# Harrypotterrrr/DVD-GAN

Hardware: AMD Instinct MI355X
Metric: clips/sec per G+Ds+Dt step, 48x64x64 UCF-101 synth (higher is better)
Workload: dtype bf16; 1 GPU; UCF-101-shaped 101-class 48x64x64 clips, G+Ds+Dt hinge step, ch=32, k_sample=8, batch 64/GPU (BASELINE configs[1]); global_batch=64, parallelism=dp1

## Files before the change

### dvd_gan_amd/csrc/conv_common.h

```cpp
#pragma once
#include "common.h"

namespace dvdk {

constexpr int BM = 128, BN = 128, NT = 256;
constexpr int TILEB = BM * 80;
constexpr int WG_LD = 132;

__device__ __forceinline__ u32x4 relu16_f32(u32x4 v) {
    v.x = (int32_t)v.x < 0 ? 0u : v.x; v.y = (int32_t)v.y < 0 ? 0u : v.y;
    v.z = (int32_t)v.z < 0 ? 0u : v.z; v.w = (int32_t)v.w < 0 ? 0u : v.w;
    return v;
}
__device__ __forceinline__ uint32_t relu2_bf16(uint32_t v) {
    uint32_t m = ((v >> 15) & 0x00010001u) * 0xffffu;
    return v & ~m;
}
__device__ __forceinline__ u32x4 relu16_bf16(u32x4 v) {
    v.x = relu2_bf16(v.x); v.y = relu2_bf16(v.y); v.z = relu2_bf16(v.z); v.w = relu2_bf16(v.w);
    return v;
}
template <typename T> __device__ __forceinline__ u32x4 relu16(u32x4 v);
template <> __device__ __forceinline__ u32x4 relu16<float>(u32x4 v) { return relu16_f32(v); }
template <> __device__ __forceinline__ u32x4 relu16<bf16_t>(u32x4 v) { return relu16_bf16(v); }

__device__ __forceinline__ void grid_pos(int m, int H, int W, int logH, int logW, int& f, int& y, int& x) {
    if (logW >= 0) { x = m & (W - 1); y = (m >> logW) & (H - 1); f = m >> (logW + logH); }
    else { f = m / (H * W); const int r = m - f * (H * W); y = r / W; x = r - y * W; }
}

struct ConvK {
    const char* in; const char* w; const float* bias; const char* res; const char* mask;
    const char* wq;
    char* out; float* ws;
    int M, C, ldi, Cout, ldo, ldres, ldmask, res_up2;
    int T, H, W, logH, logW, Hin, Win;
    int kt, kh, kw, kchunks, nk, nsplit, tilesN;
    int up2, relu_in, act, out_f32;
    int nb32;
// ... 47 lines not shown
    a.x = pack2_bf16(v[0], v[1]); a.y = pack2_bf16(v[2], v[3]); a.z = pack2_bf16(v[4], v[5]); a.w = pack2_bf16(v[6], v[7]);
    __builtin_amdgcn_raw_buffer_store_b128(a, r, off, 0, 0);
}
template <> __device__ __forceinline__ void bst8<float>(__amdgpu_buffer_rsrc_t r, unsigned off, const float (&v)[8]) {
    u32x4 a = {__float_as_uint(v[0]), __float_as_uint(v[1]), __float_as_uint(v[2]), __float_as_uint(v[3])};
    u32x4 b = {__float_as_uint(v[4]), __float_as_uint(v[5]), __float_as_uint(v[6]), __float_as_uint(v[7])};
    __builtin_amdgcn_raw_buffer_store_b128(a, r, off, 0, 0);
    __builtin_amdgcn_raw_buffer_store_b128(b, r, off + 16, 0, 0);
}

template <int R, int D, class Stage, class Load, class Compute>
__device__ __forceinline__ void epi_run(Stage stage, Load load, Compute compute) {
#pragma unroll
    for (int i = 0; i < D && i < R; ++i) load(i);
#pragma unroll
    for (int i = 0; i < R; ++i) {
        if ((i & 3) == 0) stage(i >> 2);
        if (i + D < R) load(i + D);
        compute(i);
        if ((i & 3) == 3) __builtin_amdgcn_wave_barrier();
    }
}

template <int TM>
__device__ __forceinline__ bool splitk_combine(const ConvK& p, f32x16 (&acc)[TM][2], float* lds0, int lane, int z, int ltile) {
    constexpr unsigned kWaveBytes = TM * 2 * 4 * 1024;
    constexpr int kSc1 = 16;
    const int ns = p.nsplit;
    const int wave = threadIdx.x >> 6;
    const unsigned tileBytes = (blockDim.x >> 6) * kWaveBytes;
    const size_t tile = (size_t)ltile;
    const __amdgpu_buffer_rsrc_t rs = __builtin_amdgcn_make_buffer_rsrc(
        (void*)((char*)p.g.slabs + tile * ns * (size_t)tileBytes), 0, (unsigned)ns * tileBytes, 0x00020000);
    const unsigned lo = wave * kWaveBytes + lane * 16;
#pragma unroll
    for (int tm = 0; tm < TM; ++tm)
#pragma unroll
        for (int tn = 0; tn < 2; ++tn)
#pragma unroll
            for (int q = 0; q < 4; ++q) {
                const u32x4 v = {__float_as_uint(acc[tm][tn][4 * q]), __float_as_uint(acc[tm][tn][4 * q + 1]),
                                 __float_as_uint(acc[tm][tn][4 * q + 2]), __float_as_uint(acc[tm][tn][4 * q + 3])};
                __builtin_amdgcn_raw_buffer_store_b128(v, rs, z * tileBytes + lo + ((tm * 2 + tn) * 4 + q) * 1024, 0, kSc1);
            }
    asm volatile("s_waitcnt vmcnt(0)" ::: "memory");
    __syncthreads();
    if (threadIdx.x == 0)
        *reinterpret_cast<volatile unsigned*>(lds0) =
            __hip_atomic_fetch_add(p.g.tickets + tile, 1u, __ATOMIC_RELAXED, __HIP_MEMORY_SCOPE_AGENT);
    __syncthreads();
    const unsigned ticket = *reinterpret_cast<volatile unsigned*>(lds0);
    if (ticket != (unsigned)(ns - 1)) return false;
    __syncthreads();
    if (threadIdx.x == 0) __hip_atomic_store(p.g.tickets + tile, 0u, __ATOMIC_RELAXED, __HIP_MEMORY_SCOPE_AGENT);
    int s_begin = 0, s_end = ns;
    if (ns == 2) { s_begin = z ^ 1; s_end = s_begin + 1; }
    else {
        const f32x16 zacc = {0.f, 0.f, 0.f, 0.f, 0.f, 0.f, 0.f, 0.f, 0.f, 0.f, 0.f, 0.f, 0.f, 0.f, 0.f, 0.f};
#pragma unroll
        for (int tm = 0; tm < TM; ++tm)
#pragma unroll
            for (int tn = 0; tn < 2; ++tn) acc[tm][tn] = zacc;
    }
    u32x4 buf[2][4];
    auto issue = [&](int s, int g, u32x4 (&b)[4]) __attribute__((always_inline)) {
        const unsigned so = s < s_end ? (unsigned)s * tileBytes : kOOB;
#pragma unroll
        for (int i = 0; i < 4; ++i) b[i] = __builtin_amdgcn_raw_buffer_load_b128(rs, so + lo + (g * 4 + i) * 1024, 0, kSc1);
    };
    issue(s_begin, 0, buf[0]);
    for (int s = s_begin; s < s_end; ++s) {
#pragma unroll
        for (int g = 0; g < 2 * TM; ++g) {
            if (g + 1 < 2 * TM) issue(s, g + 1, buf[(g + 1) & 1]);
            else issue(s + 1, 0, buf[(g + 1) & 1]);
            __builtin_amdgcn_sched_barrier(0);
#pragma unroll
            for (int i = 0; i < 4; ++i) {
                const u32x4 v = buf[g & 1][i];
                f32x16& a = acc[g >> 1][g & 1];
                a[4 * i] += __uint_as_float(v.x); a[4 * i + 1] += __uint_as_float(v.y);
                a[4 * i + 2] += __uint_as_float(v.z); a[4 * i + 3] += __uint_as_float(v.w);
            }
            __builtin_amdgcn_sched_barrier(0);
        }
    }
    return true;
}

template <typename T, int TM, int DEEP = 0, bool COMBINE = true, class RelRow>
__device__ __forceinline__ void conv_epilogue(const ConvK& p, f32x16 (&acc)[TM][2], float* ep, int lane, int col, int z, int ltile,
                                              long long row0, RelRow relrow) {
    constexpr unsigned esz = sizeof(T);
    constexpr int R = 4 * TM;
    constexpr bool kB = sizeof(T) == 2;
    const int erow = lane >> 3, ecol = (lane & 7) * 8;
    const bool colv = col < p.Cout;
    const long long rows = (long long)p.M - row0;
    auto stage = [&](int tm) __attribute__((always_inline)) {
#pragma unroll
        for (int tn = 0; tn < 2; ++tn)
#pragma unroll
            for (int r = 0; r < 16; ++r)
                ep[((r & 3) + 8 * (r >> 2) + 4 * (lane >> 5)) * 64 + tn * 32 + (lane & 31)] = acc[tm][tn][r];
        __builtin_amdgcn_s_waitcnt(0xc07f);
        __builtin_amdgcn_wave_barrier();
    };
    auto staged = [&](int i, float (&v)[8]) __attribute__((always_inline)) {
        const f32x4 a = *reinterpret_cast<const f32x4*>(ep + ((i & 3) * 8 + erow) * 64 + ecol);
        const f32x4 b = *reinterpret_cast<const f32x4*>(ep + ((i & 3) * 8 + erow) * 64 + ecol + 4);
        v[0] = a[0]; v[1] = a[1]; v[2] = a[2]; v[3] = a[3]; v[4] = b[0]; v[5] = b[1]; v[6] = b[2]; v[7] = b[3];
    };
    auto rrow = [&](int i) __attribute__((always_inline)) -> int { return relrow(i >> 2, i & 3); };
    auto offs = [&](int rr, unsigned ld, unsigned eb, int c, bool ok) __attribute__((always_inline)) -> unsigned {
        return (rr >= 0 && ok) ? (unsigned)rr * (ld * eb) + (unsigned)c * eb : kOOB;
    };
    const int mode = p.g.mode;
#ifdef DVD_EXP_NOEPI
    return;
#endif
    if constexpr (COMBINE)
        if (mode != 0 && p.nsplit > 1 && !splitk_combine<TM>(p, acc, ep - (threadIdx.x >> 6) * (32 * 64), lane, z, ltile)) return;
    if (mode == 1) {
        constexpr int D = kB ? 3 : 1;
        const int h = p.g.h;
        const bool isr = col >= h;
        const int c2 = isr ? col - h : col;
// ... 286 lines not shown
```

### dvd_gan_amd/csrc/conv_gb.hip

```cpp
#include "conv_common.h"

namespace {

#ifndef DVD_GB_EPI_DEEP
#define DVD_GB_EPI_DEEP 0
#endif

constexpr unsigned kRowOOB = 0x80000000u, kStepOOB = 0x40000000u, kRangeCap = 0x3fffffffu;

template <int TM, int WN, int WMV, bool UP2> struct HaloGbCfg {
    static constexpr int PITCH = HaloGeo<UP2>::PITCH;
    static constexpr int NWAVE = WMV * WN;
    static constexpr int PH = WMV * TM * 2;
    static constexpr int HG = UP2 ? ((PH / 2 + 3) * PITCH + 15) / 16 : ((PH + 4) * PITCH + 15) / 16;
    static constexpr int HBYTES = HG * 1024;
    static constexpr int EPI = NWAVE * 32 * 64 * 4;
    static constexpr int LDSB = 2 * HBYTES + 1024 > EPI ? 2 * HBYTES + 1024 : EPI;
};

template <int TM, bool RELU, class LdA, class Next>
__device__ __forceinline__ void gb_step(f32x16 (&acc)[TM][2], const bf16x8 (&b)[2][2], LdA ldA, Next next) {
    constexpr int NU = 2 * TM;
#ifndef DVD_GB_ADEPTH
#define DVD_GB_ADEPTH 2
#endif
    constexpr int AD = DVD_GB_ADEPTH;
    bf16x8 a[NU];
#pragma unroll
    for (int u = 0; u < AD && u < NU; ++u) a[u] = ldA(u);
    __builtin_amdgcn_sched_barrier(0);
#pragma unroll
    for (int u = 0; u < NU; ++u) {
        if (u + AD < NU) a[u + AD] = ldA(u + AD);
        const int kk = u / TM, tm = u % TM;
        if constexpr (RELU) a[u] = __builtin_bit_cast(bf16x8, relu16_bf16(__builtin_bit_cast(u32x4, a[u])));
#pragma unroll
        for (int tn = 0; tn < 2; ++tn)
            acc[tm][tn] = __builtin_amdgcn_mfma_f32_32x32x16_bf16(a[u], b[kk][tn], acc[tm][tn], 0, 0, 0);
        __builtin_amdgcn_sched_barrier(0);
        if (u == 0) {
#ifndef DVD_EXP_NODMA
            next();
#endif
            __builtin_amdgcn_sched_barrier(0);
        }
    }
}

template <int TM, int WN, int WMV, bool RELU, bool UP2, int KS>
__device__ __forceinline__ void conv_halo_gb_tile(const ConvK& p, char* const smem, const int mt, const int nt, const int z, const int ltile) {
    using T = bf16_t;
    using G = HaloGeo<UP2>;
    using Cfg = HaloGbCfg<TM, WN, WMV, UP2>;
    constexpr int NWAVE = Cfg::NWAVE;
    constexpr int PITCH = G::PITCH;
    constexpr int BNt = WN * 64;
    constexpr int PH = Cfg::PH, HG = Cfg::HG, HBYTES = Cfg::HBYTES;
    constexpr int NH = (HG + NWAVE - 1) / NWAVE;
    constexpr int ntap2 = KS * KS;
    constexpr int pad = KS >> 1, cpad = (pad + 1) >> 1;
    constexpr int HWa = UP2 ? ((15 + pad) >> 1) + cpad + 1 : 16 + 2 * pad;
    constexpr int HHa = UP2 ? ((PH - 1 + pad) >> 1) + cpad + 1 : PH + 2 * pad;
    char* const hbuf0 = &smem[0];
    char* const dump = &smem[2 * HBYTES];
    const int tid = threadIdx.x, lane = tid & 63, wave = tid >> 6;
    const int wm = wave / WN, wn = wave % WN;
    const int n0 = nt * BNt;
    const int pw = p.W >> 4, ppf = pw * (p.H / PH);
    const int ft = mt / ppf, pidx = mt - ft * ppf;
    const int y0 = (pidx / pw) * PH, x0 = (pidx % pw) * 16;
    const int nouter = p.kchunks * p.kt;
    const int per = (nouter + p.nsplit - 1) / p.nsplit;
    const int oc_begin = z * per, oc_end = min(nouter, oc_begin + per);
    constexpr unsigned esz = 2;
    const int iy_lo = UP2 ? (y0 >> 1) - cpad : y0 - pad, ix_lo = UP2 ? (x0 >> 1) - cpad : x0 - pad;

    const int wu = __builtin_amdgcn_readfirstlane(wave);
    const int lrow = lane >> 2;
    const unsigned ldb = (unsigned)p.ldi * esz;
    const int tt = p.kt > 1 ? ft % p.T : 0;
    const int base_frame = max(0, ft - (p.kt >> 1));
    const size_t fbytes = (size_t)p.Hin * p.Win * ldb;
    const size_t base_b = (size_t)base_frame * fbytes;
    const size_t left_b = p.in_bytes - base_b;
    const __amdgpu_buffer_rsrc_t rin = __builtin_amdgcn_make_buffer_rsrc(
        (void*)(p.in + base_b), 0, left_b > kRangeCap ? kRangeCap : (unsigned)left_b, 0x00020000);
    const int nb32 = p.nb32;
    const __amdgpu_buffer_rsrc_t rwq = __builtin_amdgcn_make_buffer_rsrc(
        (void*)p.wq, 0, (unsigned)((size_t)p.kt * ntap2 * p.kchunks * nb32 * 2048), 0x00020000);
    auto hrow = [&](int i, int& hy, int& hx) __attribute__((always_inline)) {
        const int h = (i * NWAVE + wu) * 16 + lrow;
        hy = h / PITCH; hx = h - hy * PITCH;
    };
    unsigned hoff[NH];
#pragma unroll
    for (int i = 0; i < NH; ++i) {
        const int g = i * NWAVE + wu;
        int hy, hx;
        hrow(i, hy, hx);
        const int yin = iy_lo + hy, xin = ix_lo + hx;
        const int hq = (lane & 3) ^ G::sw(hy, hx);
        const bool ok = g < HG && hy < HHa && hx < HWa && (unsigned)yin < (unsigned)p.Hin && (unsigned)xin < (unsigned)p.Win;
        hoff[i] = ok ? (unsigned)(yin * p.Win + xin) * ldb + hq * 16 : kRowOOB;
    }
    const bool ragged = (p.C & 31) != 0;
    auto dmaH = [&](int hb, int cc_, int it_) __attribute__((always_inline)) {
        const int dt_ = it_ - (p.kt >> 1);
        const bool ok_ = (unsigned)(tt + dt_) < (unsigned)p.T || p.kt == 1;
        const unsigned ud_ = ok_ ? (unsigned)(ft + dt_ - base_frame) * (unsigned)fbytes + cc_ * 64 : kStepOOB;
        const bool part_ = ragged && cc_ == p.kchunks - 1;
#pragma unroll
        for (int i = 0; i < NH; ++i) {
            const int g = i * NWAVE + wu;
            char* dst_ = g < HG ? hbuf0 + hb * HBYTES + g * 1024 : dump;
            unsigned off_ = hoff[i] + ud_;
            if (part_) {
                int hy, hx;
                hrow(i, hy, hx);
                const int hq = (lane & 3) ^ G::sw(hy, hx);
                off_ = cc_ * 32 + hq * 8 < p.C ? off_ : kRowOOB;
            }
            dma16(rin, dst_, off_);
        }
    };
    const unsigned bvoff = (unsigned)(wn * 2 * 2048 + lane * 16);
    const unsigned bnt = (unsigned)(nt * (BNt / 32)) * 2048u;
    const unsigned brec = (unsigned)nb32 * 2048u;
    const unsigned tapstep = (unsigned)p.kchunks * brec;
    auto ldBq = [&](bf16x8 (&b)[2][2], unsigned rec) __attribute__((always_inline)) {
#pragma unroll
        for (int kk = 0; kk < 2; ++kk)
#pragma unroll
            for (int tn = 0; tn < 2; ++tn)
                b[kk][tn] = __builtin_bit_cast(bf16x8, __builtin_amdgcn_raw_buffer_load_b128(rwq, bvoff, rec + (unsigned)(tn * 2048 + kk * 1024), 0));
    };
    auto rec0 = [&](int cc_, int it_) __attribute__((always_inline)) -> unsigned {
        return ((unsigned)(it_ * ntap2) * p.kchunks + cc_) * brec + bnt;
    };

    f32x16 acc[TM][2];
    {
        const f32x16 zacc = {0.f, 0.f, 0.f, 0.f, 0.f, 0.f, 0.f, 0.f, 0.f, 0.f, 0.f, 0.f, 0.f, 0.f, 0.f, 0.f};
#pragma unroll
        for (int a = 0; a < TM; ++a)
#pragma unroll
            for (int b = 0; b < 2; ++b) acc[a][b] = zacc;
    }
    const int l31 = lane & 31, kh2 = lane >> 5;
    const int px = l31 & 15, py0 = wm * (TM * 2) + (l31 >> 4);
    constexpr int TMSTRIDE = (UP2 ? 1 : 2) * PITCH * 64;
#ifdef DVD_EXP_NOMAIN
    const int nouter_z = 0;
#else
    const int nouter_z = oc_end - oc_begin;
#endif
    if (nouter_z > 0) {
        int m_cc = oc_begin / p.kt, m_it = oc_begin - m_cc * p.kt;
        int h_cc = m_cc, h_it = m_it;
        bf16x8 bq0[2][2], bq1[2][2];
        unsigned rec = rec0(m_cc, m_it);
        dmaH(0, h_cc, h_it);
        if (++h_it == p.kt) { h_it = 0; ++h_cc; }
        ldBq(bq0, rec);
        __builtin_amdgcn_s_waitcnt(0x0070 | (0xf << 8));
        __builtin_amdgcn_s_barrier();
        int hb = 0, iy = 0, left = nouter_z;
        auto row = [&](bf16x8 (&b0)[2][2], bf16x8 (&b1)[2][2]) __attribute__((always_inline)) {
            const bool first = iy == 0, last = iy == KS - 1, more = left > 1;
            const int hy = UP2 ? ((py0 + iy - pad) >> 1) + cpad : py0 + iy;
            const char* const Arow = hbuf0 + hb * HBYTES + hy * (PITCH * 64);
#pragma unroll
            for (int ix = 0; ix < KS; ++ix) {
                const int hx = UP2 ? ((px + ix - pad) >> 1) + cpad : px + ix;
                const int swz = G::sw(hy, hx);
                const char* const Ah = Arow + hx * 64;
                auto ldA = [&](int u) __attribute__((always_inline)) -> bf16x8 {
                    const int kk = u / TM, tm = u % TM, slot = kk * 2 + kh2;
                    const int sl = (UP2 && (tm & 1)) ? (slot ^ 2) : slot;
                    return *reinterpret_cast<const bf16x8*>(Ah + tm * TMSTRIDE + ((sl ^ swz) << 4));
                };
                unsigned nrec = rec + tapstep;
                if (ix == KS - 1 && last) {
                    int n_cc = m_cc, n_it = m_it + 1;
                    if (n_it == p.kt) { n_it = 0; ++n_cc; }
                    nrec = more ? rec0(n_cc, n_it) : rec;
                    m_cc = n_cc; m_it = n_it;
                }
                auto next = [&]() __attribute__((always_inline)) {
                    ldBq((ix & 1) ? b0 : b1, nrec);
                    if (ix == 0 && first && more) { dmaH(hb ^ 1, h_cc, h_it); if (++h_it == p.kt) { h_it = 0; ++h_cc; } }
                };
                gb_step<TM, RELU>(acc, (ix & 1) ? b1 : b0, ldA, next);
                rec = nrec;
            }
            ++iy;
            if (last) {
                iy = 0; hb ^= 1; --left;
                if (more) {
#ifndef DVD_EXP_NOWAIT
                    __builtin_amdgcn_s_waitcnt(0xc07f);
#endif
#ifndef DVD_EXP_NOBAR
                    __builtin_amdgcn_s_barrier();
#endif
                }
            }
        };
        const int nrows = nouter_z * KS;
        int r = 0;
#pragma unroll 1
        for (; r + 1 < nrows; r += 2) { row(bq0, bq1); row(bq1, bq0); }
        if (r < nrows) row(bq0, bq1);
    }
    __syncthreads();

    float* ep = reinterpret_cast<float*>(&smem[0]) + wave * (32 * 64);
    const int ecol = (lane & 7) * 8, erow = lane >> 3;
    const long long frame_row0 = (long long)ft * (p.H * p.W);
    conv_epilogue<T, TM, DVD_GB_EPI_DEEP>(p, acc, ep, lane, n0 + wn * 64 + ecol, z, ltile, frame_row0, [&](int tm, int j) __attribute__((always_inline)) {
        const int pi = wm * (TM * 32) + tm * 32 + j * 8 + erow;
        return (y0 + (pi >> 4)) * p.W + x0 + (pi & 15);
    });
}

__device__ __forceinline__ int xcd_order(int bid, int nwg) {
    const int xcd = bid & 7, qd = nwg >> 3, rr = nwg & 7;
    return (xcd < rr ? xcd * (qd + 1) : rr * (qd + 1) + (xcd - rr) * qd) + (bid >> 3);
}
struct TileMN { int mt, nt; };
__device__ __forceinline__ TileMN tile_of(int nmajor, int tilesN, int t, int ntiles) {
    const int d = nmajor ? ntiles / tilesN : tilesN;
    const int q = t / d, r = t - q * d;
    TileMN o;
    o.mt = nmajor ? r : q; o.nt = nmajor ? q : r;
    return o;
}

template <int TM, int WN, int WMV, bool RELU, bool UP2, int KS>
__global__ __launch_bounds__(256, 2) void conv_halo_gb_kernel(ConvK p) {
    __shared__ __attribute__((aligned(16))) char smem[HaloGbCfg<TM, WN, WMV, UP2>::LDSB];
    const int bid = xcd_order(blockIdx.x, gridDim.x);
    const TileMN t = tile_of(p.nmajor, p.tilesN, bid, gridDim.x);
    conv_halo_gb_tile<TM, WN, WMV, RELU, UP2, KS>(p, smem, t.mt, t.nt, blockIdx.z, (int)blockIdx.x);
}

template <int TM, int S> struct HaloGbsCfg {
    static constexpr int PITCH = S + 4, FR = PITCH * PITCH;
    static constexpr int G = TM * 64 / (S * S);
    static constexpr int HG = (G * FR + 15) / 16;
    static constexpr int HBYTES = HG * 1024;
    static constexpr int EPI = 4 * 32 * 64 * 4;
    static constexpr int LDSB = 2 * HBYTES + 1024 > EPI ? 2 * HBYTES + 1024 : EPI;
};

template <int TM, int S, bool RELU, int KS>
__device__ __forceinline__ void conv_halo_gbs_tile(const ConvK& p, char* const smem, const int mt, const int nt, const int z, const int ltile) {
    using T = bf16_t;
    using Cfg = HaloGbsCfg<TM, S>;
    constexpr int WN = 2, NWAVE = 4, BNt = 128;
    constexpr int PITCH = Cfg::PITCH, FR = Cfg::FR, G = Cfg::G, HG = Cfg::HG, HBYTES = Cfg::HBYTES;
    constexpr int NH = (HG + NWAVE - 1) / NWAVE;
    constexpr int SS = S * S;
    constexpr int ntap2 = KS * KS, pad = KS >> 1, ext = S + 2 * pad;
    char* const hbuf0 = &smem[0];
    char* const dump = &smem[2 * HBYTES];
    const int tid = threadIdx.x, lane = tid & 63, wave = tid >> 6;
    const int wm = wave / WN, wn = wave % WN;
    const int n0 = nt * BNt;
    const int ft0 = mt * G, nframes = p.M / SS;
    const int per = (p.kchunks + p.nsplit - 1) / p.nsplit;
    const int cc_begin = z * per, cc_end = min(p.kchunks, cc_begin + per);
    constexpr unsigned esz = 2;

    const int wu = __builtin_amdgcn_readfirstlane(wave);
    const int lrow = lane >> 2;
    const unsigned ldb = (unsigned)p.ldi * esz;
    const size_t base_b = (size_t)ft0 * SS * ldb;
    const size_t left_b = p.in_bytes - base_b;
    const __amdgpu_buffer_rsrc_t rin = __builtin_amdgcn_make_buffer_rsrc(
        (void*)(p.in + base_b), 0, left_b > kRangeCap ? kRangeCap : (unsigned)left_b, 0x00020000);
    const int nb32 = p.nb32;
    const __amdgpu_buffer_rsrc_t rwq = __builtin_amdgcn_make_buffer_rsrc(
        (void*)p.wq, 0, (unsigned)((size_t)ntap2 * p.kchunks * nb32 * 2048), 0x00020000);
    auto hrow = [&](int i, int& fl, int& hy, int& hx) __attribute__((always_inline)) {
        const int h = (i * NWAVE + wu) * 16 + lrow;
        fl = h / FR;
        const int r = h - fl * FR;
        hy = r / PITCH; hx = r - hy * PITCH;
    };
    unsigned hoff[NH];
#pragma unroll
    for (int i = 0; i < NH; ++i) {
        const int g = i * NWAVE + wu;
        int fl, hy, hx;
        hrow(i, fl, hy, hx);
        const int yin = hy - pad, xin = hx - pad;
        const int hq = (lane & 3) ^ (hy & 3);
        const bool ok = g < HG && fl < G && ft0 + fl < nframes && hy < ext && hx < ext && (unsigned)yin < (unsigned)S && (unsigned)xin < (unsigned)S;
        hoff[i] = ok ? (unsigned)((fl * S + yin) * S + xin) * ldb + hq * 16 : kRowOOB;
    }
    const bool ragged = (p.C & 31) != 0;
    auto dmaH = [&](int hb, int cc_) __attribute__((always_inline)) {
        const bool part_ = ragged && cc_ == p.kchunks - 1;
#pragma unroll
        for (int i = 0; i < NH; ++i) {
            const int g = i * NWAVE + wu;
            char* dst_ = g < HG ? hbuf0 + hb * HBYTES + g * 1024 : dump;
            unsigned off_ = hoff[i] + cc_ * 64;
            if (part_) {
                int fl, hy, hx;
                hrow(i, fl, hy, hx);
                const int hq = (lane & 3) ^ (hy & 3);
                off_ = cc_ * 32 + hq * 8 < p.C ? off_ : kRowOOB;
            }
            dma16(rin, dst_, off_);
        }
    };
    const unsigned bvoff = (unsigned)(wn * 2 * 2048 + lane * 16);
    const unsigned bnt = (unsigned)(nt * (BNt / 32)) * 2048u;
    const unsigned brec = (unsigned)nb32 * 2048u;
    const unsigned tapstep = (unsigned)p.kchunks * brec;
    auto ldBq = [&](bf16x8 (&b)[2][2], unsigned rec) __attribute__((always_inline)) {
#pragma unroll
        for (int kk = 0; kk < 2; ++kk)
#pragma unroll
            for (int tn = 0; tn < 2; ++tn)
                b[kk][tn] = __builtin_bit_cast(bf16x8, __builtin_amdgcn_raw_buffer_load_b128(rwq, bvoff, rec + (unsigned)(tn * 2048 + kk * 1024), 0));
    };

    f32x16 acc[TM][2];
    {
        const f32x16 zacc = {0.f, 0.f, 0.f, 0.f, 0.f, 0.f, 0.f, 0.f, 0.f, 0.f, 0.f, 0.f, 0.f, 0.f, 0.f, 0.f};
#pragma unroll
        for (int a = 0; a < TM; ++a)
#pragma unroll
            for (int b = 0; b < 2; ++b) acc[a][b] = zacc;
    }
    const int l31 = lane & 31, kh2 = lane >> 5;
    const int pi0 = wm * (TM * 32) + l31;
    const int f0 = pi0 / SS, y0 = (pi0 % SS) / S, x0 = pi0 % S;
    const int arow0 = f0 * FR + y0 * PITCH + x0;
    auto tmoff = [](int tm) constexpr -> int { return S == 8 ? ((tm >> 1) * FR + (tm & 1) * 4 * PITCH) * 64 : tm * 2 * FR * 64; };
#ifdef DVD_EXP_NOMAIN
    const int nch = 0;
#else
    const int nch = cc_end - cc_begin;
#endif
    if (nch > 0) {
        unsigned rec = (unsigned)cc_begin * brec + bnt;
        bf16x8 bq0[2][2], bq1[2][2];
        dmaH(0, cc_begin);
        ldBq(bq0, rec);
        __builtin_amdgcn_s_waitcnt(0x0070 | (0xf << 8));
        __builtin_amdgcn_s_barrier();
        int hb = 0, iy = 0, cc = cc_begin;
        auto row = [&](bf16x8 (&b0)[2][2], bf16x8 (&b1)[2][2]) __attribute__((always_inline)) {
            const bool first = iy == 0, last = iy == KS - 1, more = cc + 1 < cc_end;
            const int swz = (y0 + iy) & 3;
            const char* const Arow = hbuf0 + hb * HBYTES + (arow0 + iy * PITCH) * 64;
#pragma unroll
            for (int ix = 0; ix < KS; ++ix) {
                const char* const Ah = Arow + ix * 64;
                auto ldA = [&](int u) __attribute__((always_inline)) -> bf16x8 {
                    const int kk = u / TM, tm = u % TM, slot = kk * 2 + kh2;
                    return *reinterpret_cast<const bf16x8*>(Ah + tmoff(tm) + ((slot ^ swz) << 4));
                };
                unsigned nrec = rec + tapstep;
                if (ix == KS - 1 && last) nrec = more ? (unsigned)(cc + 1) * brec + bnt : rec;
                auto next = [&]() __attribute__((always_inline)) {
                    ldBq((ix & 1) ? b0 : b1, nrec);
                    if (ix == 0 && first && more) dmaH(hb ^ 1, cc + 1);
                };
                gb_step<TM, RELU>(acc, (ix & 1) ? b1 : b0, ldA, next);
                rec = nrec;
            }
            ++iy;
            if (last) {
                iy = 0; hb ^= 1; ++cc;
                if (more) {
                    __builtin_amdgcn_s_waitcnt(0xc07f);
                    __builtin_amdgcn_s_barrier();
                }
            }
        };
        const int nrows = nch * KS;
        int r = 0;
#pragma unroll 1
        for (; r + 1 < nrows; r += 2) { row(bq0, bq1); row(bq1, bq0); }
        if (r < nrows) row(bq0, bq1);
    }
    __syncthreads();

    float* ep = reinterpret_cast<float*>(&smem[0]) + wave * (32 * 64);
    const int ecol = (lane & 7) * 8, erow = lane >> 3;
    const long long row0 = (long long)ft0 * SS;
    conv_epilogue<T, TM, DVD_GB_EPI_DEEP>(p, acc, ep, lane, n0 + wn * 64 + ecol, z, ltile, row0, [&](int tm, int j) __attribute__((always_inline)) {
        const int pi = wm * (TM * 32) + tm * 32 + j * 8 + erow;
        return row0 + pi < p.M ? pi : -1;
    });
}

template <int TM, int S, bool RELU, int KS>
__global__ __launch_bounds__(256, 2) void conv_halo_gbs_kernel(ConvK p) {
    __shared__ __attribute__((aligned(16))) char smem[HaloGbsCfg<TM, S>::LDSB];
    const int bid = xcd_order(blockIdx.x, gridDim.x);
    const TileMN t = tile_of(p.nmajor, p.tilesN, bid, gridDim.x);
    conv_halo_gbs_tile<TM, S, RELU, KS>(p, smem, t.mt, t.nt, blockIdx.z, (int)blockIdx.x);
}

template <class TileFn>
__device__ __forceinline__ void group_dispatch(const ConvGroup& grp, TileFn fn) {
    const int x = blockIdx.x & 7;
    int rem = blockIdx.x >> 3;
    auto share = [&](int m) __attribute__((always_inline)) -> int { const int w = grp.wgs[m]; return (w >> 3) + (x < (w & 7) ? 1 : 0); };
    const int m0 = grp.order[0], m1 = grp.n > 1 ? grp.order[1] : m0;
    const int s0 = share(m0), s1 = grp.n > 1 ? share(m1) : 0;
    const int h0 = min(grp.head, s0), h1 = min(grp.head, s1);
    int g = -1, off = 0;
    if (rem < h0) { g = m0; off = rem; }
    else if ((rem -= h0) < h1) { g = m1; off = rem; }
    else if ((rem -= h1) < s0 - h0) { g = m0; off = h0 + rem; }
    else if ((rem -= s0 - h0) < s1 - h1) { g = m1; off = h1 + rem; }
    else {
        rem -= s1 - h1;
        for (int k = 2; k < grp.n; ++k) {
            const int m = grp.order[k], s = share(m);
            if (rem < s) { g = m; off = rem; break; }
            rem -= s;
        }
    }
    if (g < 0) return;
    const int w = grp.wgs[g];
    const int local = x * (w >> 3) + min(x, w & 7) + off;
    const ConvK& p = grp.c[g];
    const int t = local / p.nsplit, z = local - t * p.nsplit;
    const TileMN mn = tile_of(p.nmajor, p.tilesN, t, w / p.nsplit);
    fn(p, mn.mt, mn.nt, z, t);
}

template <int TM, int WN, int WMV>
__global__ __launch_bounds__(256, 2) void conv_group_gb_kernel(ConvGroup grp) {
    __shared__ __attribute__((aligned(16))) char smem[HaloGbCfg<TM, WN, WMV, false>::LDSB];
    group_dispatch(grp, [&](const ConvK& p, int mt, int nt, int z, int t) __attribute__((always_inline)) {
        if (p.kh == 5) conv_halo_gb_tile<TM, WN, WMV, false, false, 5>(p, smem, mt, nt, z, t);
        else conv_halo_gb_tile<TM, WN, WMV, false, false, 3>(p, smem, mt, nt, z, t);
    });
}

template <int TM, int S>
__global__ __launch_bounds__(256, 2) void conv_group_gbs_kernel(ConvGroup grp) {
    __shared__ __attribute__((aligned(16))) char smem[HaloGbsCfg<TM, S>::LDSB];
    group_dispatch(grp, [&](const ConvK& p, int mt, int nt, int z, int t) __attribute__((always_inline)) {
        if (p.kh == 5) conv_halo_gbs_tile<TM, S, false, 5>(p, smem, mt, nt, z, t);
        else conv_halo_gbs_tile<TM, S, false, 3>(p, smem, mt, nt, z, t);
    });
}

}

namespace dvdk {
#define GB(R, C, KS, RL, UP) cv_key(CV_HALO_L2, 0, R, C, KS, RL, UP)
#define GBS(F, R, KS, RL) cv_key(F, 0, R, 128, KS, RL, 0)
static const ConvRow kGbRows[] = {
#ifdef DVD_GB_PROBE
    {GB(256, 128, 5, 0, 0), conv_halo_gb_kernel<4, 2, 2, false, false, 5>}, {GBS(CV_FRAME8, 128, 3, 0), conv_halo_gbs_kernel<2, 8, false, 3>},
#else
    {GB(256, 128, 3, 0, 0), conv_halo_gb_kernel<4, 2, 2, false, false, 3>}, {GB(256, 128, 3, 1, 0), conv_halo_gb_kernel<4, 2, 2, true, false, 3>},
    {GB(256, 128, 3, 0, 1), conv_halo_gb_kernel<4, 2, 2, false, true, 3>},  {GB(256, 128, 3, 1, 1), conv_halo_gb_kernel<4, 2, 2, true, true, 3>},
    {GB(256, 128, 5, 0, 0), conv_halo_gb_kernel<4, 2, 2, false, false, 5>}, {GB(256, 128, 5, 1, 0), conv_halo_gb_kernel<4, 2, 2, true, false, 5>},
    {GB(256, 128, 5, 0, 1), conv_halo_gb_kernel<4, 2, 2, false, true, 5>},  {GB(256, 128, 5, 1, 1), conv_halo_gb_kernel<4, 2, 2, true, true, 5>},
    {GB(128, 128, 3, 0, 0), conv_halo_gb_kernel<2, 2, 2, false, false, 3>}, {GB(128, 128, 3, 1, 0), conv_halo_gb_kernel<2, 2, 2, true, false, 3>},
    {GB(128, 128, 3, 0, 1), conv_halo_gb_kernel<2, 2, 2, false, true, 3>},  {GB(128, 128, 3, 1, 1), conv_halo_gb_kernel<2, 2, 2, true, true, 3>},
    {GB(128, 128, 5, 0, 0), conv_halo_gb_kernel<2, 2, 2, false, false, 5>}, {GB(128, 128, 5, 1, 0), conv_halo_gb_kernel<2, 2, 2, true, false, 5>},
// ... 27 lines not shown
```

Before: 146.4 clips/s.

## Switch halo conv kernels from 32x32x16 to 16x16x32 MFMA with remapped fragment rows

Replaces the 32x32x16 bf16 MFMA in the halo conv mainloops with 16x16x32 MFMA, using a compile-time row-permutation type that maps fragment rows to pixel positions. The A/B load addressing, accumulator layout, epilogue staging and split-k combine paths are made generic over the new accumulator type. It also raises launch-bounds occupancy to 3 blocks for small-TM variants, recomputes halo offsets on the fly for relu TM=4 to save registers, and uses packed i16 max for the bf16 relu. The goal is better MFMA throughput and occupancy, at the cost of more intricate layout logic and possible register pressure or LDS bank conflicts.

```diff
diff --git a/dvd_gan_amd/csrc/conv_common.h b/dvd_gan_amd/csrc/conv_common.h
--- a/dvd_gan_amd/csrc/conv_common.h
+++ b/dvd_gan_amd/csrc/conv_common.h
@@ -12,9 +12,9 @@
     v.z = (int32_t)v.z < 0 ? 0u : v.z; v.w = (int32_t)v.w < 0 ? 0u : v.w;
     return v;
 }
+typedef __attribute__((ext_vector_type(2))) short i16x2;
 __device__ __forceinline__ uint32_t relu2_bf16(uint32_t v) {
-    uint32_t m = ((v >> 15) & 0x00010001u) * 0xffffu;
-    return v & ~m;
+    return __builtin_bit_cast(uint32_t, __builtin_elementwise_max(__builtin_bit_cast(i16x2, v), i16x2{0, 0}));
 }
 __device__ __forceinline__ u32x4 relu16_bf16(u32x4 v) {
     v.x = relu2_bf16(v.x); v.y = relu2_bf16(v.y); v.z = relu2_bf16(v.z); v.w = relu2_bf16(v.w);
@@ -108,8 +108,68 @@
     }
 }
 
-template <int TM>
-__device__ __forceinline__ bool splitk_combine(const ConvK& p, f32x16 (&acc)[TM][2], float* lds0, int lane, int z, int ltile) {
+template <int B0, int B1, int B2, int B3, int B4> struct FragRows {
+    static constexpr int bit(int rid, int b) { return (rid >> b) & 1; }
+    static constexpr int pix(int h, int i) {
+        const int rid = h << 4 | i;
+        return bit(rid, B0) | bit(rid, B1) << 1 | bit(rid, B2) << 2 | bit(rid, B3) << 3 | bit(rid, B4) << 4;
+    }
+};
+using RowsHalo = FragRows<0, 1, 4, 2, 3>;
+using RowsUp2 = FragRows<0, 2, 3, 4, 1>;
+using RowsF8 = FragRows<0, 1, 2, 4, 3>;
+template <class Rows> struct Acc16 { f32x4 q[2][4]; };
+
+__device__ __forceinline__ void acc_zero(f32x16 (&t)[2]) {
+    const f32x16 z = {0.f, 0.f, 0.f, 0.f, 0.f, 0.f, 0.f, 0.f, 0.f, 0.f, 0.f, 0.f, 0.f, 0.f, 0.f, 0.f};
+    t[0] = z; t[1] = z;
+}
+template <class Rows> __device__ __forceinline__ void acc_zero(Acc16<Rows>& a) {
+    const f32x4 z = {0.f, 0.f, 0.f, 0.f};
+#pragma unroll
+    for (int g = 0; g < 8; ++g) a.q[g >> 2][g & 3] = z;
+}
+__device__ __forceinline__ u32x4 acc_quad(const f32x16 (&t)[2], int g) {
+    const f32x16& a = t[g >> 2];
+    const int q = g & 3;
+    return u32x4{__float_as_uint(a[4 * q]), __float_as_uint(a[4 * q + 1]), __float_as_uint(a[4 * q + 2]), __float_as_uint(a[4 * q + 3])};
+}
+template <class Rows> __device__ __forceinline__ u32x4 acc_quad(const Acc16<Rows>& a, int g) { return __builtin_bit_cast(u32x4, a.q[g >> 2][g & 3]); }
+__device__ __forceinline__ void acc_add(f32x16 (&t)[2], int g, u32x4 v) {
+    f32x16& a = t[g >> 2];
+    const int q = g & 3;
+    a[4 * q] += __uint_as_float(v.x); a[4 * q + 1] += __uint_as_float(v.y);
+    a[4 * q + 2] += __uint_as_float(v.z); a[4 * q + 3] += __uint_as_float(v.w);
+}
+template <class Rows> __device__ __forceinline__ void acc_add(Acc16<Rows>& a, int g, u32x4 v) {
+    f32x4& x = a.q[g >> 2][g & 3];
+    x[0] += __uint_as_float(v.x); x[1] += __uint_as_float(v.y); x[2] += __uint_as_float(v.z); x[3] += __uint_as_float(v.w);
+}
+__device__ __forceinline__ void acc_stage(const f32x16 (&t)[2], float* ep, int lane) {
+#pragma unroll
+    for (int tn = 0; tn < 2; ++tn)
+#pragma unroll
+        for (int r = 0; r < 16; ++r)
+            ep[((r & 3) + 8 * (r >> 2) + 4 * (lane >> 5)) * 64 + tn * 32 + (lane & 31)] = t[tn][r];
+}
+template <class Rows> __device__ __forceinline__ void acc_stage(const Acc16<Rows>& a, float* ep, int lane) {
+    const int kg = lane >> 4;
+    const bool odd = kg & 1;
+    float* const e0 = ep + Rows::pix(0, 4 * kg) * 64 + (lane & 15) + (odd ? 16 : 0);
+    float* const e1 = ep + Rows::pix(0, 4 * kg) * 64 + (lane & 15) + (odd ? 0 : 16);
+#pragma unroll
+    for (int h = 0; h < 2; ++h)
+#pragma unroll
+        for (int j = 0; j < 4; ++j) {
+#pragma unroll
+            for (int r = 0; r < 4; ++r)
+                ((j & 1) ? e1 : e0)[Rows::pix(h, r) * 64 + (j >> 1) * 32] = odd ? a.q[h][j ^ 1][r] : a.q[h][j][r];
+            __builtin_amdgcn_sched_barrier(0);
+        }
+}
+
+template <int TM, class Acc>
+__device__ __forceinline__ bool splitk_combine(const ConvK& p, Acc (&acc)[TM], float* lds0, int lane, int z, int ltile) {
     constexpr unsigned kWaveBytes = TM * 2 * 4 * 1024;
     constexpr int kSc1 = 16;
     const int ns = p.nsplit;
@@ -122,13 +182,8 @@
 #pragma unroll
     for (int tm = 0; tm < TM; ++tm)
 #pragma unroll
-        for (int tn = 0; tn < 2; ++tn)
-#pragma unroll
-            for (int q = 0; q < 4; ++q) {
-                const u32x4 v = {__float_as_uint(acc[tm][tn][4 * q]), __float_as_uint(acc[tm][tn][4 * q + 1]),
-                                 __float_as_uint(acc[tm][tn][4 * q + 2]), __float_as_uint(acc[tm][tn][4 * q + 3])};
-                __builtin_amdgcn_raw_buffer_store_b128(v, rs, z * tileBytes + lo + ((tm * 2 + tn) * 4 + q) * 1024, 0, kSc1);
-            }
+        for (int g = 0; g < 8; ++g)
+            __builtin_amdgcn_raw_buffer_store_b128(acc_quad(acc[tm], g), rs, z * tileBytes + lo + (tm * 8 + g) * 1024, 0, kSc1);
     asm volatile("s_waitcnt vmcnt(0)" ::: "memory");
     __syncthreads();
     if (threadIdx.x == 0)
@@ -142,11 +197,8 @@
     int s_begin = 0, s_end = ns;
     if (ns == 2) { s_begin = z ^ 1; s_end = s_begin + 1; }
     else {
-        const f32x16 zacc = {0.f, 0.f, 0.f, 0.f, 0.f, 0.f, 0.f, 0.f, 0.f, 0.f, 0.f, 0.f, 0.f, 0.f, 0.f, 0.f};
-#pragma unroll
-        for (int tm = 0; tm < TM; ++tm)
-#pragma unroll
-            for (int tn = 0; tn < 2; ++tn) acc[tm][tn] = zacc;
+#pragma unroll
+        for (int tm = 0; tm < TM; ++tm) acc_zero(acc[tm]);
     }
     u32x4 buf[2][4];
     auto issue = [&](int s, int g, u32x4 (&b)[4]) __attribute__((always_inline)) {
@@ -162,20 +214,15 @@
             else issue(s + 1, 0, buf[(g + 1) & 1]);
             __builtin_amdgcn_sched_barrier(0);
 #pragma unroll
-            for (int i = 0; i < 4; ++i) {
-                const u32x4 v = buf[g & 1][i];
-                f32x16& a = acc[g >> 1][g & 1];
-                a[4 * i] += __uint_as_float(v.x); a[4 * i + 1] += __uint_as_float(v.y);
-                a[4 * i + 2] += __uint_as_float(v.z); a[4 * i + 3] += __uint_as_float(v.w);
-            }
+            for (int i = 0; i < 4; ++i) acc_add(acc[g >> 1], (g & 1) * 4 + i, buf[g & 1][i]);
             __builtin_amdgcn_sched_barrier(0);
         }
     }
     return true;
 }
 
-template <typename T, int TM, int DEEP = 0, bool COMBINE = true, class RelRow>
-__device__ __forceinline__ void conv_epilogue(const ConvK& p, f32x16 (&acc)[TM][2], float* ep, int lane, int col, int z, int ltile,
+template <typename T, int TM, int DEEP = 0, bool COMBINE = true, class Acc, class RelRow>
+__device__ __forceinline__ void conv_epilogue(const ConvK& p, Acc (&acc)[TM], float* ep, int lane, int col, int z, int ltile,
                                               long long row0, RelRow relrow) {
     constexpr unsigned esz = sizeof(T);
     constexpr int R = 4 * TM;
@@ -184,11 +231,7 @@
     const bool colv = col < p.Cout;
     const long long rows = (long long)p.M - row0;
     auto stage = [&](int tm) __attribute__((always_inline)) {
-#pragma unroll
-        for (int tn = 0; tn < 2; ++tn)
-#pragma unroll
-            for (int r = 0; r < 16; ++r)
-                ep[((r & 3) + 8 * (r >> 2) + 4 * (lane >> 5)) * 64 + tn * 32 + (lane & 31)] = acc[tm][tn][r];
+        acc_stage(acc[tm], ep, lane);
         __builtin_amdgcn_s_waitcnt(0xc07f);
         __builtin_amdgcn_wave_barrier();
     };
diff --git a/dvd_gan_amd/csrc/conv_gb.hip b/dvd_gan_amd/csrc/conv_gb.hip
--- a/dvd_gan_amd/csrc/conv_gb.hip
+++ b/dvd_gan_amd/csrc/conv_gb.hip
@@ -9,6 +9,8 @@
 constexpr unsigned kRowOOB = 0x80000000u, kStepOOB = 0x40000000u, kRangeCap = 0x3fffffffu;
 
 template <int TM, int WN, int WMV, bool UP2> struct HaloGbCfg {
+    using Rows = std::conditional_t<UP2, RowsUp2, RowsHalo>;
+    static_assert(Rows::pix(1, 0) == (UP2 ? 8 : 4), "fragment 1 = fragment 0 moved 4 footprint columns");
     static constexpr int PITCH = HaloGeo<UP2>::PITCH;
     static constexpr int NWAVE = WMV * WN;
     static constexpr int PH = WMV * TM * 2;
@@ -18,13 +20,13 @@
     static constexpr int LDSB = 2 * HBYTES + 1024 > EPI ? 2 * HBYTES + 1024 : EPI;
 };
 
-template <int TM, bool RELU, class LdA, class Next>
-__device__ __forceinline__ void gb_step(f32x16 (&acc)[TM][2], const bf16x8 (&b)[2][2], LdA ldA, Next next) {
+template <int TM, bool RELU, class Rows, class LdA, class Next>
+__device__ __forceinline__ void gb_step(Acc16<Rows> (&acc)[TM], const bf16x8 (&b)[4], LdA ldA, Next next) {
     constexpr int NU = 2 * TM;
 #ifndef DVD_GB_ADEPTH
 #define DVD_GB_ADEPTH 2
 #endif
-    constexpr int AD = DVD_GB_ADEPTH;
+    constexpr int AD = (RELU && TM == 4) ? 1 : DVD_GB_ADEPTH;
     bf16x8 a[NU];
 #pragma unroll
     for (int u = 0; u < AD && u < NU; ++u) a[u] = ldA(u);
@@ -32,11 +34,11 @@
 #pragma unroll
     for (int u = 0; u < NU; ++u) {
         if (u + AD < NU) a[u + AD] = ldA(u + AD);
-        const int kk = u / TM, tm = u % TM;
+        const int tm = u >> 1, h = u & 1;
         if constexpr (RELU) a[u] = __builtin_bit_cast(bf16x8, relu16_bf16(__builtin_bit_cast(u32x4, a[u])));
 #pragma unroll
-        for (int tn = 0; tn < 2; ++tn)
-            acc[tm][tn] = __builtin_amdgcn_mfma_f32_32x32x16_bf16(a[u], b[kk][tn], acc[tm][tn], 0, 0, 0);
+        for (int j = 0; j < 4; ++j)
+            acc[tm].q[h][j] = __builtin_amdgcn_mfma_f32_16x16x32_bf16(a[u], b[j], acc[tm].q[h][j], 0, 0, 0);
         __builtin_amdgcn_sched_barrier(0);
         if (u == 0) {
 #ifndef DVD_EXP_NODMA
@@ -52,6 +54,7 @@
     using T = bf16_t;
     using G = HaloGeo<UP2>;
     using Cfg = HaloGbCfg<TM, WN, WMV, UP2>;
+    using Rows = typename Cfg::Rows;
     constexpr int NWAVE = Cfg::NWAVE;
     constexpr int PITCH = G::PITCH;
     constexpr int BNt = WN * 64;
@@ -64,11 +67,11 @@
     char* const hbuf0 = &smem[0];
     char* const dump = &smem[2 * HBYTES];
     const int tid = threadIdx.x, lane = tid & 63, wave = tid >> 6;
-    const int wm = wave / WN, wn = wave % WN;
+    const int wm = wave / WN, wn = wave % WN, kg = lane >> 4;
     const int n0 = nt * BNt;
     const int pw = p.W >> 4, ppf = pw * (p.H / PH);
-    const int ft = mt / ppf, pidx = mt - ft * ppf;
-    const int y0 = (pidx / pw) * PH, x0 = (pidx % pw) * 16;
+    const int ft = __builtin_amdgcn_readfirstlane(mt / ppf), pidx = mt - ft * ppf;
+    const int y0 = __builtin_amdgcn_readfirstlane((pidx / pw) * PH), x0 = __builtin_amdgcn_readfirstlane((pidx % pw) * 16);
     const int nouter = p.kchunks * p.kt;
     const int per = (nouter + p.nsplit - 1) / p.nsplit;
     const int oc_begin = z * per, oc_end = min(nouter, oc_begin + per);
@@ -88,66 +91,63 @@
     const int nb32 = p.nb32;
     const __amdgpu_buffer_rsrc_t rwq = __builtin_amdgcn_make_buffer_rsrc(
         (void*)p.wq, 0, (unsigned)((size_t)p.kt * ntap2 * p.kchunks * nb32 * 2048), 0x00020000);
-    auto hrow = [&](int i, int& hy, int& hx) __attribute__((always_inline)) {
+    auto hrow = [&](int i, int lrow, int& hy, int& hx) __attribute__((always_inline)) {
         const int h = (i * NWAVE + wu) * 16 + lrow;
         hy = h / PITCH; hx = h - hy * PITCH;
     };
-    unsigned hoff[NH];
-#pragma unroll
-    for (int i = 0; i < NH; ++i) {
+    auto hoff_of = [&](int i, int ln) __attribute__((always_inline)) -> unsigned {
         const int g = i * NWAVE + wu;
         int hy, hx;
-        hrow(i, hy, hx);
+        hrow(i, ln >> 2, hy, hx);
         const int yin = iy_lo + hy, xin = ix_lo + hx;
-        const int hq = (lane & 3) ^ G::sw(hy, hx);
+        const int hq = (ln & 3) ^ G::sw(hy, hx);
         const bool ok = g < HG && hy < HHa && hx < HWa && (unsigned)yin < (unsigned)p.Hin && (unsigned)xin < (unsigned)p.Win;
-        hoff[i] = ok ? (unsigned)(yin * p.Win + xin) * ldb + hq * 16 : kRowOOB;
-    }
+        return ok ? (unsigned)(yin * p.Win + xin) * ldb + hq * 16 : kRowOOB;
+    };
+    constexpr bool REOFF = RELU && TM == 4;
+    unsigned hoff[NH];
+#pragma unroll
+    for (int i = 0; i < NH; ++i) hoff[i] = REOFF ? 0u : hoff_of(i, lane);
     const bool ragged = (p.C & 31) != 0;
     auto dmaH = [&](int hb, int cc_, int it_) __attribute__((always_inline)) {
         const int dt_ = it_ - (p.kt >> 1);
         const bool ok_ = (unsigned)(tt + dt_) < (unsigned)p.T || p.kt == 1;
         const unsigned ud_ = ok_ ? (unsigned)(ft + dt_ - base_frame) * (unsigned)fbytes + cc_ * 64 : kStepOOB;
         const bool part_ = ragged && cc_ == p.kchunks - 1;
+        int ln_ = lane;
+        if (part_ || REOFF) asm volatile("" : "+v"(ln_));
 #pragma unroll
         for (int i = 0; i < NH; ++i) {
             const int g = i * NWAVE + wu;
             char* dst_ = g < HG ? hbuf0 + hb * HBYTES + g * 1024 : dump;
-            unsigned off_ = hoff[i] + ud_;
+            unsigned off_ = (REOFF ? hoff_of(i, ln_) : hoff[i]) + ud_;
             if (part_) {
                 int hy, hx;
-                hrow(i, hy, hx);
-                const int hq = (lane & 3) ^ G::sw(hy, hx);
+                hrow(i, ln_ >> 2, hy, hx);
+                const int hq = (ln_ & 3) ^ G::sw(hy, hx);
                 off_ = cc_ * 32 + hq * 8 < p.C ? off_ : kRowOOB;
             }
             dma16(rin, dst_, off_);
         }
     };
-    const unsigned bvoff = (unsigned)(wn * 2 * 2048 + lane * 16);
+    const unsigned bvoff = (unsigned)(wn * 2 * 2048 + (kg >> 1) * 1024 + ((kg & 1) * 32 + (lane & 15)) * 16);
     const unsigned bnt = (unsigned)(nt * (BNt / 32)) * 2048u;
     const unsigned brec = (unsigned)nb32 * 2048u;
     const unsigned tapstep = (unsigned)p.kchunks * brec;
-    auto ldBq = [&](bf16x8 (&b)[2][2], unsigned rec) __attribute__((always_inline)) {
-#pragma unroll
-        for (int kk = 0; kk < 2; ++kk)
-#pragma unroll
-            for (int tn = 0; tn < 2; ++tn)
-                b[kk][tn] = __builtin_bit_cast(bf16x8, __builtin_amdgcn_raw_buffer_load_b128(rwq, bvoff, rec + (unsigned)(tn * 2048 + kk * 1024), 0));
+    auto ldBq = [&](bf16x8 (&b)[4], unsigned rec) __attribute__((always_inline)) {
+#pragma unroll
+        for (int j = 0; j < 4; ++j)
+            b[j] = __builtin_bit_cast(bf16x8, __builtin_amdgcn_raw_buffer_load_b128(rwq, bvoff, rec + (unsigned)((j >> 1) * 2048 + (j & 1) * 256), 0));
     };
     auto rec0 = [&](int cc_, int it_) __attribute__((always_inline)) -> unsigned {
         return ((unsigned)(it_ * ntap2) * p.kchunks + cc_) * brec + bnt;
     };
 
-    f32x16 acc[TM][2];
-    {
-        const f32x16 zacc = {0.f, 0.f, 0.f, 0.f, 0.f, 0.f, 0.f, 0.f, 0.f, 0.f, 0.f, 0.f, 0.f, 0.f, 0.f, 0.f};
-#pragma unroll
-        for (int a = 0; a < TM; ++a)
-#pragma unroll
-            for (int b = 0; b < 2; ++b) acc[a][b] = zacc;
-    }
-    const int l31 = lane & 31, kh2 = lane >> 5;
-    const int px = l31 & 15, py0 = wm * (TM * 2) + (l31 >> 4);
+    Acc16<Rows> acc[TM];
+#pragma unroll
+    for (int a = 0; a < TM; ++a) acc_zero(acc[a]);
+    const int pix0 = Rows::pix(0, lane & 15);
+    const int px = pix0 & 15, py0 = wm * (TM * 2) + (pix0 >> 4);
     constexpr int TMSTRIDE = (UP2 ? 1 : 2) * PITCH * 64;
 #ifdef DVD_EXP_NOMAIN
     const int nouter_z = 0;
@@ -157,7 +157,7 @@
     if (nouter_z > 0) {
         int m_cc = oc_begin / p.kt, m_it = oc_begin - m_cc * p.kt;
         int h_cc = m_cc, h_it = m_it;
-        bf16x8 bq0[2][2], bq1[2][2];
+        bf16x8 bq0[4], bq1[4];
         unsigned rec = rec0(m_cc, m_it);
         dmaH(0, h_cc, h_it);
         if (++h_it == p.kt) { h_it = 0; ++h_cc; }
@@ -165,19 +165,19 @@
         __builtin_amdgcn_s_waitcnt(0x0070 | (0xf << 8));
         __builtin_amdgcn_s_barrier();
         int hb = 0, iy = 0, left = nouter_z;
-        auto row = [&](bf16x8 (&b0)[2][2], bf16x8 (&b1)[2][2]) __attribute__((always_inline)) {
+        auto row = [&](bf16x8 (&b0)[4], bf16x8 (&b1)[4]) __attribute__((always_inline)) {
             const bool first = iy == 0, last = iy == KS - 1, more = left > 1;
             const int hy = UP2 ? ((py0 + iy - pad) >> 1) + cpad : py0 + iy;
             const char* const Arow = hbuf0 + hb * HBYTES + hy * (PITCH * 64);
 #pragma unroll
             for (int ix = 0; ix < KS; ++ix) {
                 const int hx = UP2 ? ((px + ix - pad) >> 1) + cpad : px + ix;
-                const int swz = G::sw(hy, hx);
+                const int swz[2] = {G::sw(hy, hx), G::sw(hy, hx + 4)};
                 const char* const Ah = Arow + hx * 64;
                 auto ldA = [&](int u) __attribute__((always_inline)) -> bf16x8 {
-                    const int kk = u / TM, tm = u % TM, slot = kk * 2 + kh2;
-                    const int sl = (UP2 && (tm & 1)) ? (slot ^ 2) : slot;
-                    return *reinterpret_cast<const bf16x8*>(Ah + tm * TMSTRIDE + ((sl ^ swz) << 4));
+                    const int tm = u >> 1, h = u & 1;
+                    const int sl = (UP2 && (tm & 1)) ? (kg ^ 2) : kg;
+                    return *reinterpret_cast<const bf16x8*>(Ah + tm * TMSTRIDE + h * 256 + ((sl ^ swz[h]) << 4));
                 };
                 unsigned nrec = rec + tapstep;
                 if (ix == KS - 1 && last) {
@@ -214,11 +214,14 @@
     }
     __syncthreads();
 
-    float* ep = reinterpret_cast<float*>(&smem[0]) + wave * (32 * 64);
-    const int ecol = (lane & 7) * 8, erow = lane >> 3;
+    int te = tid;
+    asm volatile("" : "+v"(te));
+    const int elane = te & 63, ewave = te >> 6, ewm = ewave / WN, ewn = ewave % WN;
+    float* ep = reinterpret_cast<float*>(&smem[0]) + ewave * (32 * 64);
+    const int ecol = (elane & 7) * 8, erow = elane >> 3;
     const long long frame_row0 = (long long)ft * (p.H * p.W);
-    conv_epilogue<T, TM, DVD_GB_EPI_DEEP>(p, acc, ep, lane, n0 + wn * 64 + ecol, z, ltile, frame_row0, [&](int tm, int j) __attribute__((always_inline)) {
-        const int pi = wm * (TM * 32) + tm * 32 + j * 8 + erow;
+    conv_epilogue<T, TM, DVD_GB_EPI_DEEP>(p, acc, ep, elane, n0 + ewn * 64 + ecol, z, ltile, frame_row0, [&](int tm, int j) __attribute__((always_inline)) {
+        const int pi = ewm * (TM * 32) + tm * 32 + j * 8 + erow;
         return (y0 + (pi >> 4)) * p.W + x0 + (pi & 15);
     });
 }
@@ -237,7 +240,7 @@
 }
 
 template <int TM, int WN, int WMV, bool RELU, bool UP2, int KS>
-__global__ __launch_bounds__(256, 2) void conv_halo_gb_kernel(ConvK p) {
+__global__ __launch_bounds__(256, TM == 2 ? 3 : 2) void conv_halo_gb_kernel(ConvK p) {
     __shared__ __attribute__((aligned(16))) char smem[HaloGbCfg<TM, WN, WMV, UP2>::LDSB];
     const int bid = xcd_order(blockIdx.x, gridDim.x);
     const TileMN t = tile_of(p.nmajor, p.tilesN, bid, gridDim.x);
@@ -245,6 +248,8 @@
 }
 
 template <int TM, int S> struct HaloGbsCfg {
+    using Rows = std::conditional_t<S == 8, RowsF8, RowsHalo>;
+    static_assert(Rows::pix(1, 0) == S, "fragment 1 = fragment 0 moved one line down");
     static constexpr int PITCH = S + 4, FR = PITCH * PITCH;
     static constexpr int G = TM * 64 / (S * S);
     static constexpr int HG = (G * FR + 15) / 16;
@@ -257,6 +262,7 @@
 __device__ __forceinline__ void conv_halo_gbs_tile(const ConvK& p, char* const smem, const int mt, const int nt, const int z, const int ltile) {
     using T = bf16_t;
     using Cfg = HaloGbsCfg<TM, S>;
+    using Rows = typename Cfg::Rows;
     constexpr int WN = 2, NWAVE = 4, BNt = 128;
     constexpr int PITCH = Cfg::PITCH, FR = Cfg::FR, G = Cfg::G, HG = Cfg::HG, HBYTES = Cfg::HBYTES;
     constexpr int NH = (HG + NWAVE - 1) / NWAVE;
@@ -265,7 +271,7 @@
     char* const hbuf0 = &smem[0];
     char* const dump = &smem[2 * HBYTES];
     const int tid = threadIdx.x, lane = tid & 63, wave = tid >> 6;
-    const int wm = wave / WN, wn = wave % WN;
+    const int wm = wave / WN, wn = wave % WN, kg = lane >> 4;
     const int n0 = nt * BNt;
     const int ft0 = mt * G, nframes = p.M / SS;
     const int per = (p.kchunks + p.nsplit - 1) / p.nsplit;
@@ -282,7 +288,7 @@
     const int nb32 = p.nb32;
     const __amdgpu_buffer_rsrc_t rwq = __builtin_amdgcn_make_buffer_rsrc(
         (void*)p.wq, 0, (unsigned)((size_t)ntap2 * p.kchunks * nb32 * 2048), 0x00020000);
-    auto hrow = [&](int i, int& fl, int& hy, int& hx) __attribute__((always_inline)) {
+    auto hrow = [&](int i, int lrow, int& fl, int& hy, int& hx) __attribute__((always_inline)) {
         const int h = (i * NWAVE + wu) * 16 + lrow;
         fl = h / FR;
         const int r = h - fl * FR;
@@ -293,7 +299,7 @@
     for (int i = 0; i < NH; ++i) {
         const int g = i * NWAVE + wu;
         int fl, hy, hx;
-        hrow(i, fl, hy, hx);
+        hrow(i, lrow, fl, hy, hx);
         const int yin = hy - pad, xin = hx - pad;
         const int hq = (lane & 3) ^ (hy & 3);
         const bool ok = g < HG && fl < G && ft0 + fl < nframes && hy < ext && hx < ext && (unsigned)yin < (unsigned)S && (unsigned)xin < (unsigned)S;
@@ -302,6 +308,8 @@
     const bool ragged = (p.C & 31) != 0;
     auto dmaH = [&](int hb, int cc_) __attribute__((always_inline)) {
         const bool part_ = ragged && cc_ == p.kchunks - 1;
+        int ln_ = lane;
+        if (part_) asm volatile("" : "+v"(ln_));
 #pragma unroll
         for (int i = 0; i < NH; ++i) {
             const int g = i * NWAVE + wu;
@@ -309,35 +317,27 @@
             unsigned off_ = hoff[i] + cc_ * 64;
             if (part_) {
                 int fl, hy, hx;
-                hrow(i, fl, hy, hx);
-                const int hq = (lane & 3) ^ (hy & 3);
+                hrow(i, ln_ >> 2, fl, hy, hx);
+                const int hq = (ln_ & 3) ^ (hy & 3);
                 off_ = cc_ * 32 + hq * 8 < p.C ? off_ : kRowOOB;
             }
             dma16(rin, dst_, off_);
         }
     };
-    const unsigned bvoff = (unsigned)(wn * 2 * 2048 + lane * 16);
+    const unsigned bvoff = (unsigned)(wn * 2 * 2048 + (kg >> 1) * 1024 + ((kg & 1) * 32 + (lane & 15)) * 16);
     const unsigned bnt = (unsigned)(nt * (BNt / 32)) * 2048u;
     const unsigned brec = (unsigned)nb32 * 2048u;
     const unsigned tapstep = (unsigned)p.kchunks * brec;
-    auto ldBq = [&](bf16x8 (&b)[2][2], unsigned rec) __attribute__((always_inline)) {
-#pragma unroll
-        for (int kk = 0; kk < 2; ++kk)
-#pragma unroll
-            for (int tn = 0; tn < 2; ++tn)
-                b[kk][tn] = __builtin_bit_cast(bf16x8, __builtin_amdgcn_raw_buffer_load_b128(rwq, bvoff, rec + (unsigned)(tn * 2048 + kk * 1024), 0));
-    };
-
-    f32x16 acc[TM][2];
-    {
-        const f32x16 zacc = {0.f, 0.f, 0.f, 0.f, 0.f, 0.f, 0.f, 0.f, 0.f, 0.f, 0.f, 0.f, 0.f, 0.f, 0.f, 0.f};
-#pragma unroll
-        for (int a = 0; a < TM; ++a)
-#pragma unroll
-            for (int b = 0; b < 2; ++b) acc[a][b] = zacc;
-    }
-    const int l31 = lane & 31, kh2 = lane >> 5;
-    const int pi0 = wm * (TM * 32) + l31;
+    auto ldBq = [&](bf16x8 (&b)[4], unsigned rec) __attribute__((always_inline)) {
+#pragma unroll
+        for (int j = 0; j < 4; ++j)
+            b[j] = __builtin_bit_cast(bf16x8, __builtin_amdgcn_raw_buffer_load_b128(rwq, bvoff, rec + (unsigned)((j >> 1) * 2048 + (j & 1) * 256), 0));
+    };
+
+    Acc16<Rows> acc[TM];
+#pragma unroll
+    for (int a = 0; a < TM; ++a) acc_zero(acc[a]);
+    const int pi0 = wm * (TM * 32) + Rows::pix(0, lane & 15);
     const int f0 = pi0 / SS, y0 = (pi0 % SS) / S, x0 = pi0 % S;
     const int arow0 = f0 * FR + y0 * PITCH + x0;
     auto tmoff = [](int tm) constexpr -> int { return S == 8 ? ((tm >> 1) * FR + (tm & 1) * 4 * PITCH) * 64 : tm * 2 * FR * 64; };
@@ -348,22 +348,22 @@
 #endif
     if (nch > 0) {
         unsigned rec = (unsigned)cc_begin * brec + bnt;
-        bf16x8 bq0[2][2], bq1[2][2];
+        bf16x8 bq0[4], bq1[4];
         dmaH(0, cc_begin);
         ldBq(bq0, rec);
         __builtin_amdgcn_s_waitcnt(0x0070 | (0xf << 8));
         __builtin_amdgcn_s_barrier();
         int hb = 0, iy = 0, cc = cc_begin;
-        auto row = [&](bf16x8 (&b0)[2][2], bf16x8 (&b1)[2][2]) __attribute__((always_inline)) {
+        auto row = [&](bf16x8 (&b0)[4], bf16x8 (&b1)[4]) __attribute__((always_inline)) {
             const bool first = iy == 0, last = iy == KS - 1, more = cc + 1 < cc_end;
-            const int swz = (y0 + iy) & 3;
+            const int swz[2] = {(y0 + iy) & 3, (y0 + iy + 1) & 3};
             const char* const Arow = hbuf0 + hb * HBYTES + (arow0 + iy * PITCH) * 64;
 #pragma unroll
             for (int ix = 0; ix < KS; ++ix) {
                 const char* const Ah = Arow + ix * 64;
                 auto ldA = [&](int u) __attribute__((always_inline)) -> bf16x8 {
-                    const int kk = u / TM, tm = u % TM, slot = kk * 2 + kh2;
-                    return *reinterpret_cast<const bf16x8*>(Ah + tmoff(tm) + ((slot ^ swz) << 4));
+                    const int tm = u >> 1, h = u & 1;
+                    return *reinterpret_cast<const bf16x8*>(Ah + tmoff(tm) + h * (PITCH * 64) + ((kg ^ swz[h]) << 4));
                 };
                 unsigned nrec = rec + tapstep;
                 if (ix == KS - 1 && last) nrec = more ? (unsigned)(cc + 1) * brec + bnt : rec;
@@ -391,17 +391,20 @@
     }
     __syncthreads();
 
-    float* ep = reinterpret_cast<float*>(&smem[0]) + wave * (32 * 64);
-    const int ecol = (lane & 7) * 8, erow = lane >> 3;
+    int te = tid;
+    asm volatile("" : "+v"(te));
+    const int elane = te & 63, ewave = te >> 6, ewm = ewave / WN, ewn = ewave % WN;
+    float* ep = reinterpret_cast<float*>(&smem[0]) + ewave * (32 * 64);
+    const int ecol = (elane & 7) * 8, erow = elane >> 3;
     const long long row0 = (long long)ft0 * SS;
-    conv_epilogue<T, TM, DVD_GB_EPI_DEEP>(p, acc, ep, lane, n0 + wn * 64 + ecol, z, ltile, row0, [&](int tm, int j) __attribute__((always_inline)) {
-        const int pi = wm * (TM * 32) + tm * 32 + j * 8 + erow;
+    conv_epilogue<T, TM, DVD_GB_EPI_DEEP>(p, acc, ep, elane, n0 + ewn * 64 + ecol, z, ltile, row0, [&](int tm, int j) __attribute__((always_inline)) {
+        const int pi = ewm * (TM * 32) + tm * 32 + j * 8 + erow;
         return row0 + pi < p.M ? pi : -1;
     });
 }
 
 template <int TM, int S, bool RELU, int KS>
-__global__ __launch_bounds__(256, 2) void conv_halo_gbs_kernel(ConvK p) {
+__global__ __launch_bounds__(256, TM == 2 && S == 8 ? 3 : 2) void conv_halo_gbs_kernel(ConvK p) {
     __shared__ __attribute__((aligned(16))) char smem[HaloGbsCfg<TM, S>::LDSB];
     const int bid = xcd_order(blockIdx.x, gridDim.x);
     const TileMN t = tile_of(p.nmajor, p.tilesN, bid, gridDim.x);
@@ -439,7 +442,7 @@
 }
 
 template <int TM, int WN, int WMV>
-__global__ __launch_bounds__(256, 2) void conv_group_gb_kernel(ConvGroup grp) {
+__global__ __launch_bounds__(256, TM == 2 ? 3 : 2) void conv_group_gb_kernel(ConvGroup grp) {
     __shared__ __attribute__((aligned(16))) char smem[HaloGbCfg<TM, WN, WMV, false>::LDSB];
     group_dispatch(grp, [&](const ConvK& p, int mt, int nt, int z, int t) __attribute__((always_inline)) {
         if (p.kh == 5) conv_halo_gb_tile<TM, WN, WMV, false, false, 5>(p, smem, mt, nt, z, t);
@@ -448,7 +451,7 @@
 }
 
 template <int TM, int S>
-__global__ __launch_bounds__(256, 2) void conv_group_gbs_kernel(ConvGroup grp) {
+__global__ __launch_bounds__(256, TM == 2 && S == 8 ? 3 : 2) void conv_group_gbs_kernel(ConvGroup grp) {
     __shared__ __attribute__((aligned(16))) char smem[HaloGbsCfg<TM, S>::LDSB];
     group_dispatch(grp, [&](const ConvK& p, int mt, int nt, int z, int t) __attribute__((always_inline)) {
         if (p.kh == 5) conv_halo_gbs_tile<TM, S, false, 5>(p, smem, mt, nt, z, t);
```

Result: faster. 150.8 clips/s, median of 6 (+3.0%).
